# Bazs/structure_from_motion

Measured on NVIDIA B200. Metric: hyp x point evals/sec (fp64), higher is better.
Workload: dtype f64

## Files before the change

### structure_from_motion_b200/csrc/sfm_score.cuh

```cuda
#pragma once
#include <type_traits>

#include "sfm_device.cuh"
#include "sfm_types.h"

namespace sfm {

__device__ __forceinline__ uint32_t smem_u32(const void* p) {
    return (uint32_t)__cvta_generic_to_shared(p);
}
__device__ __forceinline__ void mbar_init(void* bar, uint32_t count) {
    asm volatile("mbarrier.init.shared::cta.b64 [%0], %1;" ::"r"(smem_u32(bar)), "r"(count) : "memory");
}
__device__ __forceinline__ void mbar_fence_init() {
    asm volatile("fence.mbarrier_init.release.cluster;" ::: "memory");
}
__device__ __forceinline__ void mbar_expect_tx(void* bar, uint32_t bytes) {
    asm volatile("mbarrier.arrive.expect_tx.shared::cta.b64 _, [%0], %1;" ::"r"(smem_u32(bar)), "r"(bytes)
                 : "memory");
}
__device__ __forceinline__ void mbar_wait(void* bar, uint32_t parity) {
    uint32_t ok;
    do {
        asm volatile(
            "{\n\t.reg .pred p;\n\t"
            "mbarrier.try_wait.parity.shared::cta.b64 p, [%1], %2;\n\t"
            "selp.u32 %0, 1, 0, p;\n\t}"
            : "=r"(ok)
            : "r"(smem_u32(bar)), "r"(parity)
            : "memory");
    } while (!ok);
}
__device__ __forceinline__ void bulk_g2s(void* dst_smem, const void* src_gmem, uint32_t bytes, void* bar) {
    asm volatile(
        "cp.async.bulk.shared::cluster.global.mbarrier::complete_tx::bytes [%0], [%1], %2, [%3];" ::"r"(
            smem_u32(dst_smem)),
        "l"(src_gmem), "r"(bytes), "r"(smem_u32(bar))
        : "memory");
}

constexpr int kScoreThreads = 128;
constexpr int kScoreWarps = kScoreThreads / 32;
constexpr int kTile = 64;
constexpr int kStages = 3;
constexpr int kRing = 64;
constexpr unsigned kMaxPoints = 1u << 25;
constexpr int kChunks = 4;
constexpr int kFixedBits = 21 * kChunks;
constexpr int kChunkBits = 21;
constexpr int kAccWords = 1 + 2 * kChunks;
constexpr long long kMaxItemPoints = 1ll << 11;
enum { SUM_S1 = 1, SUM_S2 = 2 };
enum { MODE_FULL = 0, MODE_SCREEN = 1, MODE_SCREEN32 = 2, MODE_SCREEN11 = 3 };
constexpr double kKappaCoef = 4.2e-20;
constexpr double kThrScreenFactor = 1.0 + 3e-9;
constexpr double kKappa32Coef = 1.2e-10;
constexpr double kThr32Factor = 1.0316;
constexpr double kRangeLo = 0x1p-200;
constexpr double kRangeHi = 0x1p200;


__global__ void __launch_bounds__(256) k_pad_models(const double* __restrict__ E, long long htotal, ModelRow* __restrict__ rows) {
    const long long i = blockIdx.x * (long long)blockDim.x + threadIdx.x;
    if (i >= htotal) return;
    const double* e = E + 9 * i;
    ModelRow r;
    r.a = make_double4(e[0], e[1], e[2], e[3]);
    r.b = make_double4(e[4], e[5], e[6], e[7]);
    r.c = make_double4(e[8], 0.0, 0.0, 0.0);
    rows[i] = r;
}

struct ScoreArgs {
    const Corr* pts;
    const void* spts;
    const double* bounds;
    long long n;
    const long long* offsets;
    const double* E;
    const ModelRow* rows;
    long long h;
    double thr, thr_pre, s;
    double kappa_coef;
    double kappa32_coef;
    double scale1, scale2;
    int sums;
    long long chunk;
    int hblocks, nsplit;
    long long total_items;
    long long htotal;
    unsigned* work_counter;
    unsigned long long* acc;
    const int* mode_flag;
    const double4* boxes;
};

__device__ __forceinline__ unsigned atom_add_acq_rel_shared(unsigned* p, unsigned v) {
    unsigned old;
    asm volatile("atom.acq_rel.cta.shared::cta.add.u32 %0, [%1], %2;" : "=r"(old) : "r"(smem_u32(p)), "r"(v) : "memory");
    return old;
}
__device__ __forceinline__ int scan_step(int v, int d) {
    asm volatile("{ .reg .pred p; .reg .b32 t; shfl.sync.up.b32 t|p, %0, %1, 0, 0xffffffff; @p add.s32 %0, %0, t; }"
                 : "+r"(v) : "r"(d));
    return v;
}
__device__ __forceinline__ unsigned lanemask_lt() {
    unsigned m;
    asm("mov.u32 %0, %%lanemask_lt;" : "=r"(m));
    return m;
}

__device__ __forceinline__ void chunks21(double x, double scale, unsigned (&c)[kChunks]) {
    const double t = x * scale;
    const unsigned long long v = __double2ull_rz(t);
    const double rem = t - __ull2double_rz(v);
    c[0] = (unsigned)__double2uint_rz(rem * 2097152.0);
    c[1] = (unsigned)v & 0x1fffffu;
    c[2] = (unsigned)(v >> kChunkBits) & 0x1fffffu;
    c[3] = (unsigned)(v >> (2 * kChunkBits));
}

struct __align__(16) Corr32 {
    float xa, ya, xb, yb;
};

__device__ __forceinline__ double tile_bound(const double (&e)[9], double4 box, double thr_pre, double kap) {
    const double l0 = fma(box.x, e[0], fma(box.y, e[3], e[6]));
    const double l1 = fma(box.x, e[1], fma(box.y, e[4], e[7]));
    const double m0 = fma(fabs(e[0]), box.z, fma(fabs(e[3]), box.w, fabs(l0)));
    const double m1 = fma(fabs(e[1]), box.z, fma(fabs(e[4]), box.w, fabs(l1)));
    const double t = fma(thr_pre, fma(m0, m0, m1 * m1), kap);
    return t == t ? t : __longlong_as_double(0x7ff0000000000000LL);
}

__device__ __forceinline__ unsigned long long k2_ordered(double x) {
    const unsigned long long b = (unsigned long long)__double_as_longlong(x);
    return (b >> 63) ? ~b : (b | 0x8000000000000000ull);
}
__device__ __forceinline__ double k2_unordered(unsigned long long k) {
    return __longlong_as_double((long long)((k >> 63) ? (k & 0x7fffffffffffffffull) : ~k));
}

__global__ void __launch_bounds__(256) k2_order_bbox(const Corr* __restrict__ pts, long long n,
                                                     unsigned long long* __restrict__ bb) {
    const long long i = blockIdx.x * (long long)blockDim.x + threadIdx.x;
    unsigned long long v[4] = {0ull, 0ull, 0ull, 0ull};
    if (i < n) {
        const Corr c = pts[i];
        if (c.xb == c.xb) { v[0] = ~k2_ordered(c.xb); v[2] = k2_ordered(c.xb); }
        if (c.yb == c.yb) { v[1] = ~k2_ordered(c.yb); v[3] = k2_ordered(c.yb); }
    }
#pragma unroll
    for (int k = 0; k < 4; ++k) {
#pragma unroll
        for (int d = 16; d > 0; d >>= 1) {
            const unsigned long long o = __shfl_xor_sync(0xffffffffu, v[k], d);
            v[k] = o > v[k] ? o : v[k];
        }
    }
    if ((threadIdx.x & 31) == 0 && i < n)
#pragma unroll
        for (int k = 0; k < 4; ++k) atomicMax(bb + k, v[k]);
}

__device__ __forceinline__ unsigned k2_quantise(double x, double lo, double hi) {
    const double sc = 65535.0 / (hi - lo);
    const double q = (sc > 0.0 && sc < 1e308) ? (x - lo) * sc : 0.0;
    return (unsigned)fmin(fmax(q, 0.0), 65535.0);
}
__device__ __forceinline__ unsigned k2_spread16(unsigned v) {
    v = (v | (v << 8)) & 0x00ff00ffu;
    v = (v | (v << 4)) & 0x0f0f0f0fu;
    v = (v | (v << 2)) & 0x33333333u;
    return (v | (v << 1)) & 0x55555555u;
}
__global__ void __launch_bounds__(256) k2_order_keys(const Corr* __restrict__ pts, long long n,
                                                     const unsigned long long* __restrict__ bb,
                                                     unsigned* __restrict__ keys, int* __restrict__ idx) {
    const long long i = blockIdx.x * (long long)blockDim.x + threadIdx.x;
    if (i >= n) return;
    const Corr c = pts[i];
    const unsigned qx = k2_quantise(c.xb, k2_unordered(~bb[0]), k2_unordered(bb[2]));
    const unsigned qy = k2_quantise(c.yb, k2_unordered(~bb[1]), k2_unordered(bb[3]));
    keys[i] = (k2_spread16(qy) << 1) | k2_spread16(qx);
    idx[i] = (int)i;
}

constexpr int kOrderWarps = 4;
__global__ void __launch_bounds__(32 * kOrderWarps) k2_order_gather(const Corr* __restrict__ pts, long long n,
                                                                   const int* __restrict__ idx, Corr* __restrict__ out,
                                                                   double4* __restrict__ boxes) {
    const long long t = (long long)blockIdx.x * kOrderWarps + (threadIdx.x >> 5);
    const int lane = threadIdx.x & 31;
    if (t * kTile >= n) return;
    double lo[2] = {__longlong_as_double(0x7ff0000000000000LL), __longlong_as_double(0x7ff0000000000000LL)};
    double hi[2] = {-lo[0], -lo[1]};
#pragma unroll
    for (int k = lane; k < kTile; k += 32) {
        const long long i = t * kTile + k;
        if (i < n) {
            const Corr c = pts[idx[i]];
            out[i] = c;
            lo[0] = fmin(lo[0], c.xb); hi[0] = fmax(hi[0], c.xb);
            lo[1] = fmin(lo[1], c.yb); hi[1] = fmax(hi[1], c.yb);
        }
    }
#pragma unroll
    for (int d = 16; d > 0; d >>= 1)
#pragma unroll
        for (int k = 0; k < 2; ++k) {
            lo[k] = fmin(lo[k], __shfl_xor_sync(0xffffffffu, lo[k], d));
            hi[k] = fmax(hi[k], __shfl_xor_sync(0xffffffffu, hi[k], d));
        }
    if (lane == 0) {
        double cw[4];
        bool finite = true;
#pragma unroll
        for (int k = 0; k < 2; ++k) {
            cw[k] = 0.5 * lo[k] + 0.5 * hi[k];
            cw[2 + k] = fmax(__dsub_ru(hi[k], cw[k]), __dsub_ru(cw[k], lo[k]));
            finite = finite && fabs(cw[k]) <= 1.7976931348623157e308 && fabs(cw[2 + k]) <= 1.7976931348623157e308;
        }
        boxes[t] = finite ? make_double4(cw[0], cw[1], cw[2], cw[3])
                          : make_double4(0.0, 0.0, 1.7976931348623157e308, 1.7976931348623157e308);
    }
}

constexpr int kPilotBlocks = 32;
constexpr int kPilotHyps = 64;
constexpr int kPilotPts = 1024;
constexpr double kPilotFullAbove = 0.09;
struct PilotArgs {
    const double* E;
    long long h;
    long long plen;
    double thr_pre;
    const double* bounds;
    double kappa_coef;
    const double4* boxes;
    unsigned* counters;
    int* mode_flag;
};
template <bool BOXES>
__device__ __forceinline__ void pilot_block(const Corr* __restrict__ pts, const PilotArgs& pa, int nb) {
    const long long nh = pa.h < kPilotHyps ? pa.h : kPilotHyps;
    const int hs = threadIdx.x % kPilotHyps;
    int pass = 0, tests = 0;
    if (hs < nh && pa.plen > 0) {
        const long long hyp = (pa.h / nh) * hs;
        double e[9], f2 = 0.0;
#pragma unroll
        for (int k = 0; k < 9; ++k) {
            e[k] = pa.E[9 * hyp + k];
            f2 = fma(e[k], e[k], f2);
        }
        const double kap = f2 * (pa.bounds[0] * pa.bounds[1] * pa.kappa_coef);
        const long long np = pa.plen < kPilotPts ? pa.plen : kPilotPts;
        const long long step = pa.plen / np;
        const int lanes = nb * (256 / kPilotHyps);
        Corr cs[8];
        double4 bx[8];
        int got = 0;
#pragma unroll
        for (int u = 0; u < 8; ++u) {
            const long long q = blockIdx.x * (256 / kPilotHyps) + threadIdx.x / kPilotHyps + (long long)u * lanes;
            if (q < np) {
                cs[u] = pts[q * step];
                if constexpr (BOXES) bx[u] = pa.boxes[q * step / kTile];
                got = u + 1;
            }
        }
#pragma unroll
        for (int u = 0; u < 8; ++u)
            if (u < got) {
                const double lb0 = fma(cs[u].xb, e[0], fma(cs[u].yb, e[3], e[6]));
                const double lb1 = fma(cs[u].xb, e[1], fma(cs[u].yb, e[4], e[7]));
                const double lb2 = fma(cs[u].xb, e[2], fma(cs[u].yb, e[5], e[8]));
                const double r = fma(cs[u].xa, lb0, fma(cs[u].ya, lb1, lb2));
                double t;
                if constexpr (BOXES) t = tile_bound(e, bx[u], pa.thr_pre, kap);
                else t = pa.thr_pre * fma(lb0, lb0, lb1 * lb1);
                pass += fma(r, r, -t) < 0.0 ? 1 : 0;
                tests += 1;
            }
    }
    unsigned long long v = ((unsigned long long)pass << 32) | (unsigned)tests;
#pragma unroll
    for (int d = 16; d > 0; d >>= 1) v += __shfl_xor_sync(0xffffffffu, v, d);
    __shared__ unsigned long long s_sum;
    __shared__ int s_last;
    if (threadIdx.x == 0) s_sum = 0ull;
    __syncthreads();
    if ((threadIdx.x & 31) == 0) atomicAdd(&s_sum, v);
    __syncthreads();
    if (threadIdx.x == 0) {
        unsigned long long* tot = reinterpret_cast<unsigned long long*>(pa.counters);
        atomicAdd(tot, s_sum);
        __threadfence();
        s_last = atomicAdd(pa.counters + 2, 1u) == (unsigned)(nb - 1);
        if (s_last) {
            __threadfence();
            const unsigned long long t = *reinterpret_cast<volatile unsigned long long*>(tot);
            const double rate = (unsigned)t ? (double)(t >> 32) / (double)(unsigned)t : 0.0;
            *pa.mode_flag = rate > kPilotFullAbove ? MODE_FULL : MODE_SCREEN;
        }
    }
}
__global__ void __launch_bounds__(256) k_pilot(const Corr* __restrict__ pts, const PilotArgs pa) {
    chain_enter();
    pilot_block<true>(pts, pa, gridDim.x);
}

__global__ void __launch_bounds__(256) k_screen_pts64(const Corr* __restrict__ pts, long long n, double inv_s,
                                                      Corr* __restrict__ spts, const PilotArgs pa) {
    chain_enter();
    const long long i = blockIdx.x * (long long)blockDim.x + threadIdx.x;
    if (i < n) {
        Corr c = pts[i];
        c.xa *= inv_s;
        c.ya *= inv_s;
        spts[i] = c;
    }
    if (!pa.mode_flag || blockIdx.x >= kPilotBlocks) return;
    pilot_block<false>(pts, pa, gridDim.x < kPilotBlocks ? gridDim.x : kPilotBlocks);
}

__global__ void __launch_bounds__(256) k_screen_pts32(const Corr* __restrict__ pts, long long n, double inv_s,
                                                      Corr32* __restrict__ spts) {
    const long long i = blockIdx.x * (long long)blockDim.x + threadIdx.x;
    if (i >= n) return;
    const Corr c = pts[i];
    Corr32 f;
    f.xa = (float)(c.xa * inv_s); f.ya = (float)(c.ya * inv_s); f.xb = (float)c.xb; f.yb = (float)c.yb;
    spts[i] = f;
}

template <int HPT>
struct alignas(128) ScoreWarpSmem {
    Corr tile[kStages][kTile];
    unsigned sacc[HPT][kAccWords][32];
    uint2 ring[kRing];
    unsigned short own[32];
    unsigned long long full_bar[kStages];
};
template <int HPT>
struct alignas(128) ScoreWarpSmemBox : ScoreWarpSmem<HPT> {
    double4 box[kStages];
    double kap[HPT][32];
};

constexpr int kTileFS = 32;
constexpr int kStagesFS = 3;
template <int HPT>
struct alignas(128) ScoreWarpSmemFS {
    Corr tile[kStagesFS][kTileFS];
    double model[32 * HPT][10];
    unsigned sacc[HPT][kAccWords][32];
    uint2 ring[kRing];
    unsigned long long full_bar[kStagesFS];
};

constexpr int score_min_blocks(int hpt) { return hpt == 2 ? 5 : 8; }


__device__ __forceinline__ int sign_word(double d) { return __double2hiint(d); }
__device__ __forceinline__ int sign_word(float f) { return __float_as_int(f); }

template <int HPT, int G, int MODE>
__device__ __forceinline__ void score_body(const ScoreArgs& a) {
    constexpr bool SCREEN = MODE != MODE_FULL;
    constexpr bool F32 = MODE == MODE_SCREEN32;
    constexpr bool SCALED = F32 || MODE == MODE_SCREEN11;
    using T = typename std::conditional<F32, float, double>::type;
    using P = typename std::conditional<F32, Corr32, Corr>::type;
    constexpr int NB = HPT * G;
    constexpr bool ENTRY = MODE == MODE_FULL;
    constexpr bool BOX = MODE == MODE_SCREEN;
    constexpr int TILE = ENTRY ? kTileFS : kTile;
    constexpr int STAGES = ENTRY ? kStagesFS : kStages;
    constexpr int AHEAD = ENTRY ? STAGES - 1 : STAGES;
    using WS = typename std::conditional<ENTRY, ScoreWarpSmemFS<HPT>,
                                         typename std::conditional<BOX, ScoreWarpSmemBox<HPT>, ScoreWarpSmem<HPT>>::type>::type;
    static_assert(NB <= 32 && (TILE % G) == 0 && (kTile % TILE) == 0, "a batch is at most 32 tests and divides a tile");
    static_assert(!ENTRY || HPT <= 2, "the two-sided body's bank swizzle of sacc holds two slots");
    extern __shared__ __align__(128) unsigned char score_smem[];
    const unsigned full = 0xffffffffu;
    const int lane = threadIdx.x & 31;
    const int warp = __shfl_sync(full, (int)(threadIdx.x >> 5), 0);
    const unsigned lt = lanemask_lt();
    if (a.mode_flag && (*a.mode_flag == MODE_FULL) != (MODE == MODE_FULL)) return;
    WS& ws = reinterpret_cast<WS*>(score_smem)[warp];

    if (lane == 0) {
#pragma unroll
        for (int s = 0; s < STAGES; ++s) mbar_init(&ws.full_bar[s], 1);
        mbar_fence_init();
    }
#pragma unroll
    for (int j = 0; j < HPT; ++j)
#pragma unroll
        for (int k = 0; k < kAccWords; ++k) ws.sacc[j][k][lane] = 0;
    __syncwarp();
    uint2* q = ws.ring;
    unsigned head = 0, tail = 0;
    unsigned gt = 0;
    const double abnd = a.bounds[0] * a.bounds[1];
    const double ab2 = SCREEN ? abnd * (F32 ? a.kappa32_coef : a.kappa_coef) : 0.0;

    for (;;) {
        unsigned item = 0;
        if (lane == 0) item = atomicAdd(a.work_counter, 1u);
        item = __shfl_sync(full, item, 0);
        if (item >= a.total_items) break;
        const int hw = (int)(item % (unsigned)a.hblocks);
        const unsigned rest = item / (unsigned)a.hblocks;
        const int split = (int)(rest % (unsigned)a.nsplit);
        const int pair = (int)(rest / (unsigned)a.nsplit);

        const long long pbase = a.offsets ? a.offsets[pair] : 0;
        const long long plen = a.offsets ? a.offsets[pair + 1] - pbase : a.n;
        long long begin = (long long)split * a.chunk;
        if (begin > plen) begin = plen;
        const long long end = pbase + ((begin + a.chunk < plen) ? begin + a.chunk : plen);
        begin += pbase;
        const int ntiles = (int)((end - begin + TILE - 1) / TILE);
        const long long hyp_w = (long long)hw * (32 * HPT);
        const double* Ep = a.E + 9 * (long long)pair * a.h;
        const ModelRow* Rw = a.rows + (long long)pair * a.h + hyp_w;
        const Corr* pbeg = a.pts + begin;
        const P* src = reinterpret_cast<const P*>(a.spts);
        const int box0 = (int)(begin / kTile);

        auto issue = [&](int t) {
            const int s = (int)((gt + (unsigned)t) % STAGES);
            const long long first = begin + (long long)t * TILE;
            const long long rem = end - first;
            const uint32_t bytes = (uint32_t)((rem < TILE ? rem : TILE) * sizeof(P));
            mbar_expect_tx(&ws.full_bar[s], bytes + (BOX ? (uint32_t)sizeof(double4) : 0u));
            bulk_g2s(&ws.tile[s][0], src + first, bytes, &ws.full_bar[s]);
            if constexpr (BOX) bulk_g2s(&ws.box[s], a.boxes + box0 + t, (uint32_t)sizeof(double4), &ws.full_bar[s]);
        };
        if (lane == 0) {
            for (int t = 0; t < AHEAD && t < ntiles; ++t) issue(t);
        }

        T e[HPT][9], kap[HPT], tb[HPT];
        unsigned fpat = 0u;
#pragma unroll
        for (int j = 0; j < HPT; ++j) {
            const long long hyp = hyp_w + 32 * j + lane;
            const bool real = hyp < a.h;
            double v[9], f2 = 0.0;
#pragma unroll
            for (int k = 0; k < 9; ++k) {
                v[k] = real ? Ep[9 * hyp + k] : 0.0;
                f2 = fma(v[k], v[k], f2);
            }
            if constexpr (ENTRY) {
                double2* mp = reinterpret_cast<double2*>(&ws.model[32 * j + lane][0]);
                mp[0] = make_double2(v[0], v[1]);
                mp[1] = make_double2(v[2], v[3]);
                mp[2] = make_double2(v[4], v[5]);
                mp[3] = make_double2(v[6], v[7]);
                ws.model[32 * j + lane][8] = v[8];
            }
            if (real && !(f2 >= kRangeLo && f2 * abnd <= kRangeHi)) fpat |= 1u << (HPT - 1 - j);
            const double nrm = F32 ? rsqrt(f2) : 1.0;
#pragma unroll
            for (int k = 0; k < 9; ++k) e[j][k] = (T)((SCALED && (k % 3) != 2) ? v[k] * nrm * a.s : v[k] * nrm);
            kap[j] = (T)(real ? (F32 ? ab2 : f2 * ab2) : -1.0);
            if constexpr (BOX) ws.kap[j][lane] = kap[j];
        }
        unsigned frep = 0u;
#pragma unroll
        for (int g = 0; g < G; ++g) frep |= 1u << (HPT * g);
        const unsigned fmask = fpat * frep;

        auto accumulate = [&](bool act, double sv, int slot, int owner) {
            if (act && (sv <= a.thr)) {
                unsigned ch[kChunks];
                unsigned* dst = &ws.sacc[slot][0][ENTRY ? (owner ^ (slot << 4)) : owner];
                atomicAdd(dst, 1u);
                if (a.sums & SUM_S1) {
                    chunks21(sv, a.scale1, ch);
#pragma unroll
                    for (int kk = 0; kk < kChunks; ++kk) atomicAdd(dst + 32 * (1 + kk), ch[kk]);
                }
                if (a.sums & SUM_S2) {
                    chunks21(__dmul_rn(sv, sv), a.scale2, ch);
#pragma unroll
                    for (int kk = 0; kk < kChunks; ++kk) atomicAdd(dst + 32 * (1 + kChunks + kk), ch[kk]);
                }
            }
        };
        auto survivor_sed = [&](unsigned hl, unsigned pos) -> double {
            double eo[9];
            Corr c;
            if constexpr (ENTRY) {
                const double2* mp = reinterpret_cast<const double2*>(&ws.model[hl][0]);
                const double2 m0 = mp[0], m1 = mp[1], m2 = mp[2], m3 = mp[3];
                eo[0] = m0.x; eo[1] = m0.y; eo[2] = m1.x; eo[3] = m1.y;
                eo[4] = m2.x; eo[5] = m2.y; eo[6] = m3.x; eo[7] = m3.y;
                eo[8] = ws.model[hl][8];
                c = (&ws.tile[0][0])[pos];
            } else {
                const ModelRow* er = Rw + hl;
                const double4 r0 = er->a, r1 = er->b;
                eo[0] = r0.x; eo[1] = r0.y; eo[2] = r0.z; eo[3] = r0.w;
                eo[4] = r1.x; eo[5] = r1.y; eo[6] = r1.z; eo[7] = r1.w;
                eo[8] = er->c.x;
                c = pbeg[pos];
            }
            return sed_exact(eo, c.xa, c.ya, c.xb, c.yb);
        };

        unsigned* qe = reinterpret_cast<unsigned*>(ws.ring);
        constexpr int LH = HPT == 4 ? 2 : (HPT == 2 ? 1 : 0);
        const unsigned ln = (unsigned)__popc(lt);
        auto drain_entries = [&]() {
            const unsigned navail = tail - head;
            const bool act = ln < navail;
            const unsigned en = act ? qe[(head + ln) & (kRing - 1)] : 0u;
            const int owner = (int)((en >> 14) & 31u), slot = LH ? (int)(en >> (32 - (LH ? LH : 1))) : 0;
            accumulate(act, survivor_sed((unsigned)(32 * slot + owner), en & 0x7ffu), slot, owner);
            head += navail < 32u ? navail : 32u;
            __syncwarp();
        };
        auto push_entries = [&](unsigned pm, unsigned pos0) {
            const unsigned base = (ln << 14) | pos0;
            unsigned vote;
            while ((vote = __ballot_sync(full, pm != 0u)) != 0u) {
                const unsigned top = 0x80000000u >> __clz(pm | 1u);
                const unsigned i = (unsigned)(NB - 32) + (unsigned)__clz(pm | 1u);
                const unsigned en = base + __funnelshift_r(i, i, LH);
                if (pm) qe[(tail + __popc(vote & lt)) & (kRing - 1)] = en;
                pm &= ~top;
                tail += __popc(vote);
                __syncwarp();
                if (tail - head >= 32u) drain_entries();
            }
        };

        auto drain_records = [&]() {
            const unsigned nrec = tail - head;
            uint2 rec = make_uint2(0u, 0u);
            if ((unsigned)lane < nrec) rec = q[(head + lane) & (kRing - 1)];
            const int cnt = __popc(rec.x);
            int incl = cnt;
#pragma unroll
            for (int d = 1; d < 32; d <<= 1) incl = scan_step(incl, d);
            const int total = __shfl_sync(full, incl, 31);
            const int m = total < 32 ? total : 32;
            const int excl = incl - cnt;
            const unsigned done_mask = __ballot_sync(full, (unsigned)lane < nrec && incl <= 32);
            const int ndone = __popc(done_mask);
            const bool act = lane < m;
            unsigned o = 0u;
            uint2 rj = make_uint2(0u, 0u);
            if constexpr (!ENTRY) {
                unsigned pmw = rec.x;
                for (int t = excl; pmw && t < 32; ++t) {
                    ws.own[t] = (unsigned short)(lane | ((__ffs(pmw) - 1) << 8));
                    pmw &= pmw - 1u;
                }
                __syncwarp();
                o = act ? ws.own[lane] : 0u;
                rj = q[(head + (o & 255u)) & (kRing - 1)];
                __syncwarp();
                if (lane == ndone && (unsigned)lane < nrec) q[(head + lane) & (kRing - 1)].x = pmw;
            }
            const int i = NB - 1 - (int)(o >> 8);
            const int owner = (int)(rj.y >> 27), slot = i % HPT;
            const unsigned rel = act ? (rj.y & 0x3fffffu) + (unsigned)(i / HPT) : 0u;
            accumulate(act, survivor_sed(act ? (unsigned)(32 * slot + owner) : 0u, rel), slot, owner);
            head += (unsigned)ndone;
            __syncwarp();
        };
        auto push_records = [&](unsigned vote, unsigned pm, unsigned rel0) {
            if (pm) q[(tail + __popc(vote & lt)) & (kRing - 1)] = make_uint2(pm, ((unsigned)lane << 27) | rel0);
            tail += __popc(vote);
            __syncwarp();
            while (tail - head >= 32u) drain_records();
        };
        auto drain = [&]() {
            if constexpr (ENTRY) drain_entries();
            else drain_records();
        };

        unsigned mark = tail;
        for (int t = 0; t < ntiles; ++t) {
            const unsigned gti = gt + (unsigned)t;
            const int s = (int)(gti % STAGES);
            mbar_wait(&ws.full_bar[s], (gti / STAGES) & 1u);
            const long long first = begin + (long long)t * TILE;
            const int np = (int)((end - first < TILE) ? (end - first) : TILE);
            const P* tp = reinterpret_cast<const P*>(&ws.tile[s][0]);
            if constexpr (BOX) {
                const double4 bx = ws.box[s];
#pragma unroll
                for (int j = 0; j < HPT; ++j) tb[j] = tile_bound(e[j], bx, a.thr_pre, ws.kap[j][lane]);
            }
            for (int p = 0; p < np; p += G) {
                unsigned pm = 0;
#pragma unroll
                for (int g = 0; g < G; ++g) {
                    const P c = tp[p + g];
                    T d[HPT];
                    if constexpr (BOX) {
                        double t0[HPT], t1[HPT], t2[HPT];
#pragma unroll
                        for (int j = 0; j < HPT; ++j) {
                            t0[j] = fma(c.yb, e[j][3], e[j][6]);
                            t1[j] = fma(c.yb, e[j][4], e[j][7]);
                            t2[j] = fma(c.yb, e[j][5], e[j][8]);
                        }
#pragma unroll
                        for (int j = 0; j < HPT; ++j) {
                            t0[j] = fma(c.xb, e[j][0], t0[j]);
                            t1[j] = fma(c.xb, e[j][1], t1[j]);
                            t2[j] = fma(c.xb, e[j][2], t2[j]);
                        }
#pragma unroll
                        for (int j = 0; j < HPT; ++j) t2[j] = fma(c.ya, t1[j], t2[j]);
#pragma unroll
                        for (int j = 0; j < HPT; ++j) t2[j] = fma(c.xa, t0[j], t2[j]);
#pragma unroll
                        for (int j = 0; j < HPT; ++j) d[j] = fma(t2[j], t2[j], -tb[j]);
                    } else if (SCREEN) {
                        T t0[HPT], t1[HPT], t2[HPT];
#pragma unroll
                        for (int j = 0; j < HPT; ++j) {
                            t0[j] = fma(c.yb, e[j][3], e[j][6]);
                            t1[j] = fma(c.yb, e[j][4], e[j][7]);
                            t2[j] = fma(c.yb, e[j][5], e[j][8]);
                        }
#pragma unroll
                        for (int j = 0; j < HPT; ++j) {
                            t0[j] = fma(c.xb, e[j][0], t0[j]);
                            t1[j] = fma(c.xb, e[j][1], t1[j]);
                            t2[j] = fma(c.xb, e[j][2], t2[j]);
                        }
#pragma unroll
                        for (int j = 0; j < HPT; ++j) t2[j] = fma(c.ya, t1[j], t2[j]);
#pragma unroll
                        for (int j = 0; j < HPT; ++j) t2[j] = fma(c.xa, t0[j], t2[j]);
#pragma unroll
                        for (int j = 0; j < HPT; ++j) t1[j] = fma(t1[j], t1[j], kap[j]);
#pragma unroll
                        for (int j = 0; j < HPT; ++j) t1[j] = fma(t0[j], t0[j], t1[j]);
#pragma unroll
                        for (int j = 0; j < HPT; ++j) d[j] = fma(t2[j], t2[j], -t1[j]);
                    } else if constexpr (!SCREEN) {
#pragma unroll
                        for (int j = 0; j < HPT; ++j) d[j] = sed_full_decision(e[j], c.xa, c.ya, c.xb, c.yb, a.thr_pre);
                    }
#pragma unroll
                    for (int j = 0; j < HPT; ++j) pm = __funnelshift_l((unsigned)sign_word(d[j]), pm, 1);
                }
                pm |= fmask;
                const int v = np - p;
                if (v < G) pm &= 0xffffffffu << (NB - v * HPT);
                const unsigned vote = __ballot_sync(full, pm != 0u);
                if (vote) {
                    if constexpr (ENTRY) push_entries(pm, (unsigned)(s * TILE + p));
                    else push_records(vote, pm, (unsigned)(first - begin) + (unsigned)p);
                }
            }
            if constexpr (ENTRY) {
                while ((int)(mark - head) > 0) drain();
                mark = tail;
            }
            __syncwarp();
            if (lane == 0 && t + AHEAD < ntiles) issue(t + AHEAD);
        }
        gt += (unsigned)ntiles;

        while (tail != head) drain();
#pragma unroll
        for (int j = 0; j < HPT; ++j) {
            const long long hyp = hyp_w + 32 * j + lane;
            const int col = ENTRY ? (lane ^ ((j & 1) << 4)) : lane;
            const unsigned cnt = ws.sacc[j][0][col];
            if (cnt) {
                unsigned long long* dst = a.acc + (long long)pair * a.h + hyp;
                atomicAdd(dst, (unsigned long long)cnt);
                ws.sacc[j][0][col] = 0;
#pragma unroll
                for (int k = 1; k < kAccWords; ++k) {
                    const unsigned v = ws.sacc[j][k][col];
                    if (v) {
                        atomicAdd(dst + (long long)k * a.htotal, (unsigned long long)v);
                        ws.sacc[j][k][col] = 0;
                    }
                }
            }
        }
        __syncwarp();
    }
}

template <int HPT, int G, int MODE>
__global__ void __launch_bounds__(kScoreThreads, score_min_blocks(MODE == MODE_SCREEN32 ? HPT / 2 : HPT))
k_score(const ScoreArgs a) {
    chain_enter();
    score_body<HPT, G, MODE>(a);
}

template <int HPT, int G, int SMODE>
__global__ void __launch_bounds__(kScoreThreads, score_min_blocks(HPT)) k_score_auto(const ScoreArgs a, const ScoreArgs a_full) {
    chain_enter();
    if (*a.mode_flag == MODE_FULL) score_body<HPT, G, MODE_FULL>(a_full);
    else score_body<HPT, G, SMODE>(a);
}

enum { AGG_SUM = 0, AGG_SQUARE = 1, AGG_MEAN = 2, AGG_RMS = 3 };
enum { SELECT_MIN_ERROR = 0, SELECT_MAX_INLIERS = 1, SELECT_MSAC = 2 };

__device__ __forceinline__ bool better(const Best& x, const Best& y, int mode) {
    if (y.idx < 0) return x.idx >= 0;
    if (x.idx < 0) return false;
    if (mode == SELECT_MAX_INLIERS) {
        if (x.count != y.count) return x.count > y.count;
        return x.idx < y.idx;
    }
    if (x.err != y.err) return x.err < y.err;
    return x.idx < y.idx;
}

__device__ __forceinline__ Best shfl_best(const Best& b, int src_delta) {
    Best r;
    r.err = __shfl_down_sync(0xffffffffu, b.err, src_delta);
    r.idx = __shfl_down_sync(0xffffffffu, b.idx, src_delta);
    r.count = __shfl_down_sync(0xffffffffu, b.count, src_delta);
    r.pad = 0;
    return r;
}

__device__ __forceinline__ Best block_best(Best b, int mode, Best* sm ) {
    const int lane = threadIdx.x & 31, warp = threadIdx.x >> 5;
#pragma unroll
    for (int d = 16; d > 0; d >>= 1) {
        const Best o = shfl_best(b, d);
        if (better(o, b, mode)) b = o;
    }
    if (lane == 0) sm[warp] = b;
    __syncthreads();
    if (warp == 0) {
        const int nw = (blockDim.x + 31) >> 5;
        Best x;
        if (lane < nw) x = sm[lane];
        else { x.err = 0.0; x.idx = -1; x.count = 0; x.pad = 0; }
#pragma unroll
        for (int d = 16; d > 0; d >>= 1) {
            const Best o = shfl_best(x, d);
            if (better(o, x, mode)) x = o;
        }
        b = x;
    }
    return b;
}

struct dd { double hi, lo; };
__device__ __forceinline__ void dd_add(dd& s, double x) {
    const double t = __dadd_rn(s.hi, x);
    const double bb = __dsub_rn(t, s.hi);
    const double e = __dadd_rn(__dsub_rn(s.hi, __dsub_rn(t, bb)), __dsub_rn(x, bb));
    s.hi = t;
    s.lo = __dadd_rn(s.lo, e);
}
__device__ __forceinline__ void dd_merge(dd& s, const dd& o) {
    dd_add(s, o.hi);
    s.lo = __dadd_rn(s.lo, o.lo);
    const double t = __dadd_rn(s.hi, s.lo);
    s.lo = __dsub_rn(s.lo, __dsub_rn(t, s.hi));
    s.hi = t;
}

__device__ __forceinline__ unsigned __int128 fixed_value(const unsigned long long* acc, long long stride) {
    unsigned __int128 v = 0;
#pragma unroll
    for (int k = kChunks - 1; k >= 0; --k) v = (v << kChunkBits) + acc[(long long)k * stride];
    return v;
}
__device__ __forceinline__ double u128_to_double(unsigned __int128 v) {
    const unsigned long long hi = (unsigned long long)(v >> 64), lo = (unsigned long long)v;
    return fma((double)hi, 18446744073709551616.0, (double)lo);
}

struct FinalArgs {
    const void* pts;
    const long long* offsets;
    const double* E;
    const uint8_t* valid;
    const int32_t* table;
    long long h;
    long long n;
    long long idx_offset;
    long long htotal;
    const unsigned long long* acc;
    double inv_scale1, inv_scale2;
    int sums;
    int force_rescore;
    double thr, min_extra;
    int agg, mode;
    int32_t* count_extra;
    double* S1;
    double* S2;
    double* err;
    Best* block_out;
    long long* block_inv;
    unsigned* tickets;
    Best* out;
    long long* invalid_out;
    SelectRecord* record;
    unsigned long long* rescored;
    unsigned* fitflag;
    const double* K;
};

template <int KIND> struct ExactModel;
template <> struct ExactModel<MODEL_E> {
    using Rec = Corr;
    static constexpr int kSample = 8;
    static constexpr int kStride = 9;
    double e[9];
    __device__ __forceinline__ void load(const double* m, const double*) {
#pragma unroll
        for (int k = 0; k < 9; ++k) e[k] = m[k];
    }
    __device__ __forceinline__ bool eval(const Corr& c, double thr, double& v) const {
        v = sed_exact(e, c.xa, c.ya, c.xb, c.yb);
        return v <= thr;
    }
};
template <> struct ExactModel<MODEL_H> {
    using Rec = Corr;
    static constexpr int kSample = 4;
    static constexpr int kStride = 9;
    double h[9], adj[9];
    __device__ __forceinline__ void load(const double* m, const double*) {
#pragma unroll
        for (int k = 0; k < 9; ++k) h[k] = m[k];
        homography_adj(h, adj);
    }
    __device__ __forceinline__ bool eval(const Corr& c, double thr, double& v) const {
        return transfer_exact(h, adj, c.xa, c.ya, c.xb, c.yb, thr, v);
    }
};

template <int KIND>
__device__ __forceinline__ bool finalise_one(const FinalArgs& a, const typename ExactModel<KIND>::Rec* pts, long long i,
                                             long long npts, bool valid, long long cnt, double s1, double s2,
                                             double& err_out, long long& cnt_out, double& s1_out, double& s2_out) {
    constexpr int KS = ExactModel<KIND>::kSample;
    const double msac = __dadd_rn(s1, __dmul_rn(a.thr, (double)(npts - cnt)));
    if (a.table && valid) {
        ExactModel<KIND> m;
        m.load(a.E + ExactModel<KIND>::kStride * i, a.K);
        for (int k = 0; k < KS; ++k) {
            const typename ExactModel<KIND>::Rec c = pts[a.table[8 * i + k]];
            double sv;
            if (m.eval(c, a.thr, sv)) {
                cnt -= 1;
            } else {
                s1 = __dadd_rn(s1, sv);
                s2 = __dadd_rn(s2, __dmul_rn(sv, sv));
            }
        }
    }
    const double n = (double)((a.table ? KS : 0) + cnt);
    double err;
    switch (a.agg) {
        case AGG_SUM: err = s1; break;
        case AGG_SQUARE: err = s2; break;
        case AGG_MEAN: err = s1 / n; break;
        default: err = sqrt(s2 / n); break;
    }
    if (a.mode == SELECT_MSAC) err = msac;
    err_out = err; cnt_out = cnt; s1_out = s1; s2_out = s2;
    return valid && (a.min_extra <= (double)cnt) && (err == err);
}

template <int KIND>
__global__ void __launch_bounds__(256) k_finalise(const FinalArgs a) {
    chain_enter();
    __shared__ Best sm[32];
    __shared__ int s_list[256];
    __shared__ int s_nlist;
    __shared__ dd s_dd[2][8];
    __shared__ long long s_cnt[8];
    __shared__ long long s_first;
    __shared__ int s_last;
    const int tid = threadIdx.x, lane = tid & 31, warp = tid >> 5;
    const long long li = blockIdx.x * (long long)blockDim.x + tid;
    const long long i = (long long)blockIdx.y * a.h + li;
    using Rec = typename ExactModel<KIND>::Rec;
    const Rec* pts = static_cast<const Rec*>(a.pts) + (a.offsets ? a.offsets[blockIdx.y] : 0);
    const long long npts = a.offsets ? a.offsets[blockIdx.y + 1] - a.offsets[blockIdx.y] : a.n;
    const double qnan = __longlong_as_double(0x7ff8000000000000LL);
    const double pinf = __longlong_as_double(0x7ff0000000000000LL);
    if (tid == 0) { s_nlist = 0; s_first = 0x7fffffffffffffffLL; }
    __syncthreads();
    Best b;
    b.err = 0.0; b.idx = -1; b.count = 0; b.pad = 0;
    if (li < a.h) {
        const bool valid = a.valid ? (a.valid[i] != 0) : true;
        const long long cnt = (long long)a.acc[i];
        const unsigned __int128 v1 = (a.sums & SUM_S1) ? fixed_value(a.acc + 1 * a.htotal + i, a.htotal) : 0;
        const unsigned __int128 v2 = (a.sums & SUM_S2) ? fixed_value(a.acc + (1 + kChunks) * a.htotal + i, a.htotal) : 0;
        const unsigned __int128 need = (unsigned __int128)(unsigned long long)cnt << 53;
        bool coarse = cnt > 0 && (((a.sums & SUM_S1) && v1 < need) || ((a.sums & SUM_S2) && v2 < need));
        if constexpr (KIND != MODEL_E) coarse = coarse && !((double)cnt < a.min_extra);
        if (valid && (a.force_rescore || coarse)) {
            s_list[atomicAdd(&s_nlist, 1)] = tid;
        } else {
            const double s1 = (a.sums & SUM_S1) ? u128_to_double(v1) * a.inv_scale1 : qnan;
            const double s2 = (a.sums & SUM_S2) ? u128_to_double(v2) * a.inv_scale2 : qnan;
            double err, s1o, s2o;
            long long c2;
            const bool cand = finalise_one<KIND>(a, pts, i, npts, valid, cnt, s1, s2, err, c2, s1o, s2o);
            a.count_extra[i] = valid ? (int32_t)c2 : -1;
            a.S1[i] = s1o;
            a.S2[i] = s2o;
            a.err[i] = cand ? err : pinf;
            if (cand) { b.err = err; b.idx = a.idx_offset + li; b.count = (int)c2; }
        }
    }
    __syncthreads();
    const int nlist = s_nlist;
    for (int q = 0; q < nlist; ++q) {
        const int owner = s_list[q];
        const long long hi_ = (long long)blockIdx.y * a.h + blockIdx.x * (long long)blockDim.x + owner;
        ExactModel<KIND> m;
        m.load(a.E + ExactModel<KIND>::kStride * hi_, a.K);
        dd p1{0.0, 0.0}, p2{0.0, 0.0};
        long long pc = 0;
        for (long long j = tid; j < npts; j += 256) {
            const Rec c = pts[j];
            double sv;
            if (m.eval(c, a.thr, sv)) {
                pc += 1;
                dd_add(p1, sv);
                dd_add(p2, __dmul_rn(sv, sv));
            }
        }
#pragma unroll
        for (int d = 16; d > 0; d >>= 1) {
            dd o1, o2;
            o1.hi = __shfl_xor_sync(0xffffffffu, p1.hi, d); o1.lo = __shfl_xor_sync(0xffffffffu, p1.lo, d);
            o2.hi = __shfl_xor_sync(0xffffffffu, p2.hi, d); o2.lo = __shfl_xor_sync(0xffffffffu, p2.lo, d);
            pc += __shfl_xor_sync(0xffffffffu, pc, d);
            if (lane & d) { dd t1 = o1, t2 = o2; dd_merge(t1, p1); dd_merge(t2, p2); p1 = t1; p2 = t2; }
            else { dd_merge(p1, o1); dd_merge(p2, o2); }
        }
        if (lane == 0) { s_dd[0][warp] = p1; s_dd[1][warp] = p2; s_cnt[warp] = pc; }
        __syncthreads();
        if (tid == owner) {
            dd t1 = s_dd[0][0], t2 = s_dd[1][0];
            long long c = s_cnt[0];
            for (int w = 1; w < 8; ++w) { dd_merge(t1, s_dd[0][w]); dd_merge(t2, s_dd[1][w]); c += s_cnt[w]; }
            double err, s1o, s2o;
            long long c2;
            const bool cand = finalise_one<KIND>(a, pts, hi_, npts, true, c, (a.sums & SUM_S1) ? t1.hi : qnan,
                                           (a.sums & SUM_S2) ? t2.hi : qnan, err, c2, s1o, s2o);
            a.count_extra[hi_] = (int32_t)c2;
            a.S1[hi_] = s1o;
            a.S2[hi_] = s2o;
            a.err[hi_] = cand ? err : pinf;
            if (cand) { b.err = err; b.idx = a.idx_offset + (hi_ - (long long)blockIdx.y * a.h); b.count = (int)c2; }
        }
        __syncthreads();
    }
    if (tid == 0 && nlist) atomicAdd(a.rescored, (unsigned long long)nlist);
    const bool inv = (li < a.h) && a.valid && (a.valid[i] == 0);
    const int ninv = __syncthreads_count(inv);
    if (inv) atomicMin(&s_first, a.idx_offset + li);
    b = block_best(b, a.mode, sm);
    __syncthreads();
    const int nblocks = gridDim.x;
    if (tid == 0) {
        const long long blk = (long long)blockIdx.y * nblocks + blockIdx.x;
        a.block_out[blk] = b;
        a.block_inv[2 * blk] = ninv;
        a.block_inv[2 * blk + 1] = s_first;
        __threadfence();
        s_last = (atomicAdd(&a.tickets[blockIdx.y], 1u) == (unsigned)(nblocks - 1)) ? 1 : 0;
    }
    __syncthreads();
    if (!s_last) return;
    __threadfence();
    __shared__ long long s_ninv, s_first2;
    if (tid == 0) {
        s_ninv = 0; s_first2 = 0x7fffffffffffffffLL; a.tickets[blockIdx.y] = 0;
        if (a.fitflag && blockIdx.y == 0) *a.fitflag = 0u;
    }
    __syncthreads();
    const volatile Best* blocks = a.block_out + (long long)blockIdx.y * nblocks;
    const volatile long long* binv = a.block_inv + 2 * (long long)blockIdx.y * nblocks;
    Best g;
    g.err = 0.0; g.idx = -1; g.count = 0; g.pad = 0;
    long long tn = 0, tf = 0x7fffffffffffffffLL;
    for (int k = tid; k < nblocks; k += 256) {
        Best o;
        o.err = blocks[k].err; o.idx = blocks[k].idx; o.count = blocks[k].count; o.pad = 0;
        if (better(o, g, a.mode)) g = o;
        tn += binv[2 * k];
        const long long f = binv[2 * k + 1];
        if (f < tf) tf = f;
    }
    if (tn) {
        atomicAdd((unsigned long long*)&s_ninv, (unsigned long long)tn);
        atomicMin(&s_first2, tf);
    }
    g = block_best(g, a.mode, sm);
    __syncthreads();
    if (tid == 0) {
        a.out[blockIdx.y] = g;
        a.invalid_out[2 * blockIdx.y] = s_ninv;
        a.invalid_out[2 * blockIdx.y + 1] = s_ninv ? s_first2 : -1;
        SelectRecord& r = a.record[blockIdx.y];
        r.best = g;
        r.num_invalid = s_ninv;
        r.first_invalid = s_ninv ? s_first2 : -1;
        const long long w = (long long)blockIdx.y * a.h + (g.idx >= 0 ? g.idx - a.idx_offset : 0);
        for (int k = 0; k < 9; ++k) r.E[k] = (KIND != MODEL_P && g.idx >= 0) ? a.E[ExactModel<KIND>::kStride * w + k] : 0.0;
        for (int k = 0; k < 8; ++k)
            r.sample[k] = (a.table && g.idx >= 0 && k < ExactModel<KIND>::kSample) ? a.table[8 * w + k] : -1;
    }
}

__global__ void __launch_bounds__(256) k_near_ties(const double* __restrict__ err, long long h, const SelectRecord* __restrict__ rec,
                                                   double rel_tol, int cap, long long* __restrict__ out, unsigned* __restrict__ count) {
    const double best = rec->best.err;
    if (rec->best.idx < 0) return;
    const double lim = best + fabs(best) * rel_tol;
    for (long long i = blockIdx.x * (long long)blockDim.x + threadIdx.x; i < h; i += (long long)gridDim.x * blockDim.x) {
        if (err[i] <= lim) {
            const unsigned pos = atomicAdd(count, 1u);
            if (pos < (unsigned)cap) out[pos] = i;
        }
    }
}

__global__ void k_merge_records(const SelectRecord* __restrict__ gathered, int world, int rank, long long hyps_per_rank,
                                int mode, SelectRecord* __restrict__ merged, int* __restrict__ owner_out,
                                double* __restrict__ winner_E, Best* __restrict__ local_best) {
    if (threadIdx.x || blockIdx.x) return;
    Best b;
    b.err = 0.0; b.idx = -1; b.count = 0; b.pad = 0;
    int owner = -1;
    for (int r = 0; r < world; ++r) {
        Best o = gathered[r].best;
        if (o.idx >= 0) o.idx += (long long)r * hyps_per_rank;
        if (better(o, b, mode)) { b = o; owner = r; }
    }
    merged->best = b;
    merged->num_invalid = gathered[rank].num_invalid;
    merged->first_invalid = gathered[rank].first_invalid;
    for (int k = 0; k < 9; ++k) {
        const double v = owner >= 0 ? gathered[owner].E[k] : 0.0;
        merged->E[k] = v;
        winner_E[k] = v;
    }
    for (int k = 0; k < 8; ++k) merged->sample[k] = owner >= 0 ? gathered[owner].sample[k] : -1;
    *owner_out = owner;
    Best lb = b;
    lb.idx = (owner == rank) ? gathered[rank].best.idx : -1;
    *local_best = lb;
}

__global__ void k_inlier_mask(const Corr* __restrict__ pts, long long n, const double* __restrict__ E,
                              const Best* __restrict__ best, long long idx_offset, long long hyp,
                              double thr, uint8_t* __restrict__ mask, double* __restrict__ sed) {
    const long long i = blockIdx.x * (long long)blockDim.x + threadIdx.x;
    if (i >= n) return;
    long long local = hyp;
    if (best) local = best->idx - idx_offset;
    if (local < 0) {
        mask[i] = 0;
        sed[i] = __longlong_as_double(0x7ff8000000000000LL);
        return;
    }
    double e[9];
#pragma unroll
    for (int k = 0; k < 9; ++k) e[k] = E[9 * local + k];
    const Corr c = pts[i];
    const double sv = sed_exact(e, c.xa, c.ya, c.xb, c.yb);
    sed[i] = sv;
    mask[i] = (sv <= thr) ? 1 : 0;
}

}
```

Baseline: 1107 billion.

## Drain survivor record ring one bit per lane and requeue remaining masks

Replaces the prefix-scan-plus-shared-memory ownership expansion in the record drain with a simpler scheme. Each lane takes one record, evaluates its lowest set bit, and pushes the rest of the mask back onto the ring tail. A separate tail drain uses a warp OR-reduction and shuffles to spread partial queues across lanes. The goal is fewer shared-memory round trips and less serial work per drain, at the cost of extra ring traffic from requeued masks and possibly more drain iterations for dense masks.

```diff
diff --git a/structure_from_motion_b200/csrc/sfm_score.cuh b/structure_from_motion_b200/csrc/sfm_score.cuh
--- a/structure_from_motion_b200/csrc/sfm_score.cuh
+++ b/structure_from_motion_b200/csrc/sfm_score.cuh
@@ -341,7 +341,6 @@
     Corr tile[kStages][kTile];
     unsigned sacc[HPT][kAccWords][32];
     uint2 ring[kRing];
-    unsigned short own[32];
     unsigned long long full_bar[kStages];
 };
 template <int HPT>
@@ -542,39 +541,49 @@
             }
         };
 
+        auto evaluate = [&](bool act, unsigned pm, unsigned y) {
+            const int i = NB - __ffs(pm);
+            const int owner = (int)(y >> 27), slot = i % HPT;
+            const unsigned rel = act ? (y & 0x3fffffu) + (unsigned)(i / HPT) : 0u;
+            accumulate(act, survivor_sed(act ? (unsigned)(32 * slot + owner) : 0u, rel), slot, owner);
+        };
         auto drain_records = [&]() {
-            const unsigned nrec = tail - head;
+            const uint2 rec = q[(head + lane) & (kRing - 1)];
+            const unsigned rest = rec.x & (rec.x - 1u);
+            const unsigned wb = __ballot_sync(full, rest != 0u);
+            __syncwarp();
+            if (rest) q[(tail + __popc(wb & lt)) & (kRing - 1)] = make_uint2(rest, rec.y);
+            head += 32u;
+            tail += __popc(wb);
+            evaluate(true, rec.x, rec.y);
+            __syncwarp();
+        };
+        auto drain_tail = [&]() {
+            const unsigned m = tail - head;
             uint2 rec = make_uint2(0u, 0u);
-            if ((unsigned)lane < nrec) rec = q[(head + lane) & (kRing - 1)];
+            if ((unsigned)lane < m) rec = q[(head + lane) & (kRing - 1)];
             const int cnt = __popc(rec.x);
             int incl = cnt;
 #pragma unroll
             for (int d = 1; d < 32; d <<= 1) incl = scan_step(incl, d);
-            const int total = __shfl_sync(full, incl, 31);
-            const int m = total < 32 ? total : 32;
             const int excl = incl - cnt;
-            const unsigned done_mask = __ballot_sync(full, (unsigned)lane < nrec && incl <= 32);
-            const int ndone = __popc(done_mask);
-            const bool act = lane < m;
-            unsigned o = 0u;
-            uint2 rj = make_uint2(0u, 0u);
-            if constexpr (!ENTRY) {
-                unsigned pmw = rec.x;
-                for (int t = excl; pmw && t < 32; ++t) {
-                    ws.own[t] = (unsigned short)(lane | ((__ffs(pmw) - 1) << 8));
-                    pmw &= pmw - 1u;
-                }
-                __syncwarp();
-                o = act ? ws.own[lane] : 0u;
-                rj = q[(head + (o & 255u)) & (kRing - 1)];
-                __syncwarp();
-                if (lane == ndone && (unsigned)lane < nrec) q[(head + lane) & (kRing - 1)].x = pmw;
-            }
-            const int i = NB - 1 - (int)(o >> 8);
-            const int owner = (int)(rj.y >> 27), slot = i % HPT;
-            const unsigned rel = act ? (rj.y & 0x3fffffu) + (unsigned)(i / HPT) : 0u;
-            accumulate(act, survivor_sed(act ? (unsigned)(32 * slot + owner) : 0u, rel), slot, owner);
-            head += (unsigned)ndone;
+            const unsigned starts = __reduce_or_sync(full, (cnt != 0 && excl < 32) ? 1u << excl : 0u);
+            const unsigned le = starts & ((lt << 1) | 1u);
+            const int src = __popc(le) - 1, k = lane - (31 - __clz(le));
+            unsigned pm = __shfl_sync(full, rec.x, src);
+            const unsigned y = __shfl_sync(full, rec.y, src);
+            for (int j = 0; j < k; ++j) pm &= pm - 1u;
+            unsigned rest = 0u;
+            if (incl > 32) {
+                rest = rec.x;
+                for (int t = excl; t < 32; ++t) rest &= rest - 1u;
+            }
+            const unsigned wb = __ballot_sync(full, rest != 0u);
+            __syncwarp();
+            if (rest) q[(tail + __popc(wb & lt)) & (kRing - 1)] = make_uint2(rest, rec.y);
+            head += m;
+            tail += __popc(wb);
+            evaluate(pm != 0u, pm, y);
             __syncwarp();
         };
         auto push_records = [&](unsigned vote, unsigned pm, unsigned rel0) {
@@ -585,7 +594,7 @@
         };
         auto drain = [&]() {
             if constexpr (ENTRY) drain_entries();
-            else drain_records();
+            else drain_tail();
         };
 
         unsigned mark = tail;
```

Result: faster. 1176 billion, median of 6 (+6.2%).
